# XiaRho/CMDA

Hardware: AMD Instinct MI355X
Metric: training images/sec (512x512 image+event, MiT-B5) (higher is better)
Workload: dtype bf16

## Files before the change

### cmda_amd/csrc/ce_loss.hip

```cpp
#include <cstdlib>
#include "bilinear.h"

namespace {
constexpr int kMaxClasses = 32;

template <int NC_MAX>
static __device__ __forceinline__ void upsample_scores(const float* __restrict__ lg, int b, int h, int w, int nc,
                                                       const BilinTap& ty, const BilinTap& tx, float (&s)[NC_MAX]) {
  const float* p00 = lg + ((long)(b * h + ty.i0) * w + tx.i0) * nc;
  const float* p01 = lg + ((long)(b * h + ty.i0) * w + tx.i1) * nc;
  const float* p10 = lg + ((long)(b * h + ty.i1) * w + tx.i0) * nc;
  const float* p11 = lg + ((long)(b * h + ty.i1) * w + tx.i1) * nc;
#pragma unroll
  for (int c = 0; c < NC_MAX; ++c)
    if (c < nc) s[c] = bilin_mix(p00[c], p01[c], p10[c], p11[c], tx.l0, tx.l1, ty.l0, ty.l1);
}

constexpr int kTW = 64, kTH = 8, kPatchFloats = 6144;

struct ScoreTile {
  int X0, Y0, b, tx0, ty0, ncols;
  bool staged;
};

static __device__ __forceinline__ ScoreTile stage_patch(const float* __restrict__ lg, float* __restrict__ patch, int h, int w, int H,
                                                        int W, int nc, float sh, float sw) {
  ScoreTile t;
  const int tiles_x = (W + kTW - 1) / kTW, tiles_y = (H + kTH - 1) / kTH;
  const int bt = blockIdx.x;
  t.b = bt / (tiles_x * tiles_y);
  const int r = bt - t.b * tiles_x * tiles_y;
  t.Y0 = (r / tiles_x) * kTH;
  t.X0 = (r % tiles_x) * kTW;
  const int X1 = min(t.X0 + kTW, W) - 1, Y1 = min(t.Y0 + kTH, H) - 1;
  t.tx0 = bilin_tap(t.X0, w, W, sw).i0;
  t.ty0 = bilin_tap(t.Y0, h, H, sh).i0;
  const int tx1 = bilin_tap(X1, w, W, sw).i1, ty1 = bilin_tap(Y1, h, H, sh).i1;
  t.ncols = tx1 - t.tx0 + 1;
  const int nrows = ty1 - t.ty0 + 1, rowf = t.ncols * nc;
  t.staged = rowf * nrows <= kPatchFloats;
  if (t.staged) {
    for (int rr = 0; rr < nrows; ++rr) {
      const float* src = lg + ((long)(t.b * h + t.ty0 + rr) * w + t.tx0) * nc;
      for (int k = threadIdx.x; k < rowf; k += blockDim.x) patch[rr * rowf + k] = src[k];
    }
  }
  __syncthreads();
  return t;
}

template <int NC_MAX>
static __device__ __forceinline__ void tile_scores(const ScoreTile& t, const float* __restrict__ lg, const float* __restrict__ patch,
                                                   int h, int w, int nc, const BilinTap& ty, const BilinTap& tx, float (&s)[NC_MAX]) {
  if (!t.staged) {
    upsample_scores<NC_MAX>(lg, t.b, h, w, nc, ty, tx, s);
    return;
  }
  const float* p00 = patch + ((ty.i0 - t.ty0) * t.ncols + (tx.i0 - t.tx0)) * nc;
  const float* p01 = patch + ((ty.i0 - t.ty0) * t.ncols + (tx.i1 - t.tx0)) * nc;
  const float* p10 = patch + ((ty.i1 - t.ty0) * t.ncols + (tx.i0 - t.tx0)) * nc;
  const float* p11 = patch + ((ty.i1 - t.ty0) * t.ncols + (tx.i1 - t.tx0)) * nc;
#pragma unroll
  for (int c = 0; c < NC_MAX; ++c)
    if (c < nc) s[c] = bilin_mix(p00[c], p01[c], p10[c], p11[c], tx.l0, tx.l1, ty.l0, ty.l1);
}

__global__ __launch_bounds__(256) void ce_fwd_kernel(const float* __restrict__ logits, const long long* __restrict__ label,
                                                      const float* __restrict__ weight, float* __restrict__ lse_out,
                                                      float* __restrict__ acc, int B, int h, int w, int H, int W, int nc,
                                                      int ignore_index) {
  __shared__ float red[2][4];
  __shared__ float patch[kPatchFloats];
  const float sh = (float)h / (float)H, sw = (float)w / (float)W;
  const ScoreTile t = stage_patch(logits, patch, h, w, H, W, nc, sh, sw);
  float lsum = 0.f, csum = 0.f;
  const int X = t.X0 + (threadIdx.x & (kTW - 1));
  for (int Y = t.Y0 + (threadIdx.x / kTW); Y < min(t.Y0 + kTH, H); Y += 256 / kTW) {
    if (X >= W) break;
    const long i = ((long)t.b * H + Y) * W + X;
    const BilinTap ty = bilin_tap(Y, h, H, sh), tx = bilin_tap(X, w, W, sw);
    float s[kMaxClasses];
    tile_scores<kMaxClasses>(t, logits, patch, h, w, nc, ty, tx, s);
    float mx = -INFINITY;
    int am = 0;
#pragma unroll
    for (int c = 0; c < kMaxClasses; ++c)
      if (c < nc && s[c] > mx) { mx = s[c]; am = c; }
    float se = 0.f;
#pragma unroll
    for (int c = 0; c < kMaxClasses; ++c)
      if (c < nc) se += __expf(s[c] - mx);
    const float lse = mx + __logf(se);
    if (lse_out) lse_out[i] = lse;
    const long long lab = label[i];
    if (lab != ignore_index && lab >= 0 && lab < nc) {
      float sl = 0.f;
#pragma unroll
      for (int c = 0; c < kMaxClasses; ++c)
        if (c == (int)lab) sl = s[c];
      const float wgt = weight ? weight[i] : 1.f;
      lsum += wgt * (lse - sl);
    }
    csum += ((long long)am == lab) ? 1.f : 0.f;
  }
  lsum = wave_sum(lsum);
  csum = wave_sum(csum);
  const int lane = threadIdx.x & 63, wid = threadIdx.x >> 6;
  if (lane == 0) { red[0][wid] = lsum; red[1][wid] = csum; }
  __syncthreads();
  if (threadIdx.x == 0) {
    atomicAdd(acc + 0, red[0][0] + red[0][1] + red[0][2] + red[0][3]);
    atomicAdd(acc + 1, red[1][0] + red[1][1] + red[1][2] + red[1][3]);
  }
}

__global__ void ce_bwd_kernel(const float* __restrict__ logits, const long long* __restrict__ label,
                              const float* __restrict__ weight, const float* __restrict__ lse,
                              const float* __restrict__ gscale_ptr, float gscale_mul, float* __restrict__ dlogits, int B,
                              int h, int w, int H, int W, int nc, int ignore_index) {
  const float sh = (float)h / (float)H, sw = (float)w / (float)W;
  const float ish = (float)H / (float)h, isw = (float)W / (float)w;
  const float gscale = (gscale_ptr ? *gscale_ptr : 1.f) * gscale_mul;
  const long total = (long)B * h * w;
  for (long i = (long)blockIdx.x * blockDim.x + threadIdx.x; i < total; i += (long)gridDim.x * blockDim.x) {
    const unsigned iu = (unsigned)i, tu = iu / (unsigned)w, bu = tu / (unsigned)h;
    const int x = (int)(iu - tu * (unsigned)w), y = (int)(tu - bu * (unsigned)h), b = (int)bu;
    int Y0 = (int)floorf(((float)y - 0.5f) * ish - 0.5f) - 1, Y1 = (int)ceilf(((float)y + 1.5f) * ish - 0.5f) + 1;
    int X0 = (int)floorf(((float)x - 0.5f) * isw - 0.5f) - 1, X1 = (int)ceilf(((float)x + 1.5f) * isw - 0.5f) + 1;
    if (y == 0) Y0 = 0;
    if (x == 0) X0 = 0;
    if (y == h - 1) Y1 = H - 1;
    if (x == w - 1) X1 = W - 1;
    Y0 = max(Y0, 0); X0 = max(X0, 0);
    Y1 = min(Y1, H - 1); X1 = min(X1, W - 1);
    float g[kMaxClasses];
#pragma unroll
    for (int c = 0; c < kMaxClasses; ++c) g[c] = 0.f;
    for (int Y = Y0; Y <= Y1; ++Y) {
      const BilinTap ty = bilin_tap(Y, h, H, sh);
      const float wy = (ty.i0 == y ? ty.l0 : 0.f) + (ty.i1 == y ? ty.l1 : 0.f);
      if (wy == 0.f) continue;
      for (int X = X0; X <= X1; ++X) {
        const BilinTap tx = bilin_tap(X, w, W, sw);
        const float wx = (tx.i0 == x ? tx.l0 : 0.f) + (tx.i1 == x ? tx.l1 : 0.f);
        if (wx == 0.f) continue;
        const long pi = ((long)b * H + Y) * W + X;
        const long long lab = label[pi];
        if (lab == ignore_index || lab < 0 || lab >= nc) continue;
        const float coef = wy * wx * (weight ? weight[pi] : 1.f);
        if (coef == 0.f) continue;
        float s[kMaxClasses];
        upsample_scores<kMaxClasses>(logits, b, h, w, nc, ty, tx, s);
        const float l = lse[pi];
#pragma unroll
        for (int c = 0; c < kMaxClasses; ++c)
          if (c < nc) g[c] += coef * (__expf(s[c] - l) - (c == (int)lab ? 1.f : 0.f));
      }
    }
    float* o = dlogits + i * nc;
#pragma unroll
    for (int c = 0; c < kMaxClasses; ++c)
      if (c < nc) o[c] = gscale * g[c];
  }
}

constexpr int kMaxTapsX = 16;

static __device__ __forceinline__ void lo_hi_range(int y, int h, int H, float ish, int& Y0, int& Y1) {
  Y0 = (int)floorf(((float)y - 0.5f) * ish - 0.5f) - 1;
  Y1 = (int)ceilf(((float)y + 1.5f) * ish - 0.5f) + 1;
  if (y == 0) Y0 = 0;
  if (y == h - 1) Y1 = H - 1;
  Y0 = max(Y0, 0);
  Y1 = min(Y1, H - 1);
}

static __device__ __forceinline__ void lo_hi_window(int y, int h, int H, float ish, int f, int& Y0, int& Y1) {
  if (f == 0) {
    lo_hi_range(y, h, H, ish, Y0, Y1);
    return;
  }
  Y0 = y == 0 ? 0 : f * y - (f >> 1);
  Y1 = y == h - 1 ? H - 1 : f * y + f + (f >> 1) - 1;
  Y0 = max(Y0, 0);
  Y1 = min(Y1, H - 1);
}

__global__ __launch_bounds__(256) void ce_bwd_gather_kernel(const float* __restrict__ logits, const long long* __restrict__ label,
                                                            const float* __restrict__ weight, const float* __restrict__ lse,
                                                            const float* __restrict__ gscale_ptr, float gscale_mul,
                                                            float* __restrict__ dlogits, int B, int h, int w, int H, int W,
                                                            int nc, int ignore_index) {
  const long total = (long)B * h * w * nc;
  const long i = (long)blockIdx.x * blockDim.x + threadIdx.x;
  if (i >= total) return;
  const float sh = (float)h / (float)H, sw = (float)w / (float)W;
  const float ish = (float)H / (float)h, isw = (float)W / (float)w;
  const unsigned iu = (unsigned)i, pu = iu / (unsigned)nc, tu = pu / (unsigned)w, bu = tu / (unsigned)h;
  const int c = (int)(iu - pu * (unsigned)nc), x = (int)(pu - tu * (unsigned)w), y = (int)(tu - bu * (unsigned)h), b = (int)bu;
  int Y0, Y1, X0, X1;
  lo_hi_range(y, h, H, ish, Y0, Y1);
  lo_hi_range(x, w, W, isw, X0, X1);
  float wxs[kMaxTapsX], lx0[kMaxTapsX], lx1[kMaxTapsX];
  unsigned sel0 = 0, sel1 = 0;
  const int nX = X1 - X0 + 1;
#pragma unroll
  for (int k = 0; k < kMaxTapsX; ++k) {
    wxs[k] = 0.f; lx0[k] = 0.f; lx1[k] = 0.f;
    if (k < nX) {
      const BilinTap tx = bilin_tap(X0 + k, w, W, sw);
      wxs[k] = (tx.i0 == x ? tx.l0 : 0.f) + (tx.i1 == x ? tx.l1 : 0.f);
      lx0[k] = tx.l0;
      lx1[k] = tx.l1;
      sel0 |= (tx.i0 == x ? 1u : 0u) << k;
      sel1 |= (tx.i1 == x ? 1u : 0u) << k;
    }
  }
  const int xm = max(x - 1, 0), xp = min(x + 1, w - 1);
  const float* Lb = logits + (long)b * h * w * nc + c;
  float g = 0.f;
  for (int Y = Y0; Y <= Y1; ++Y) {
    const BilinTap ty = bilin_tap(Y, h, H, sh);
    const float wy = (ty.i0 == y ? ty.l0 : 0.f) + (ty.i1 == y ? ty.l1 : 0.f);
    if (wy == 0.f) continue;
    const float* r0 = Lb + (long)ty.i0 * w * nc;
    const float* r1 = Lb + (long)ty.i1 * w * nc;
    const float a0 = r0[(long)xm * nc], a1 = r0[(long)x * nc], a2 = r0[(long)xp * nc];
    const float b0 = r1[(long)xm * nc], b1 = r1[(long)x * nc], b2 = r1[(long)xp * nc];
    const long rowp = ((long)b * H + Y) * W + X0;
#pragma unroll
    for (int k = 0; k < kMaxTapsX; ++k) {
      if (k >= nX || wxs[k] == 0.f) continue;
      const long long lab = label[rowp + k];
      if (lab == ignore_index || lab < 0 || lab >= nc) continue;
      const float coef = wy * wxs[k] * (weight ? weight[rowp + k] : 1.f);
      if (coef == 0.f) continue;
      const bool s0 = (sel0 >> k) & 1u, s1 = (sel1 >> k) & 1u;
      const float sc = bilin_mix(s0 ? a1 : a0, s1 ? a1 : a2, s0 ? b1 : b0, s1 ? b1 : b2, lx0[k], lx1[k], ty.l0, ty.l1);
      g += coef * (__expf(sc - lse[rowp + k]) - (c == (int)lab ? 1.f : 0.f));
    }
  }
  dlogits[i] = (gscale_ptr ? *gscale_ptr : 1.f) * gscale_mul * g;
}

constexpr int kTLW = 8, kTLH = 4, kStripRows = 8, kStripCols = 48, kStripFloats = kStripRows * kStripCols * 20;
constexpr int kLowPatchFloats = (kTLW + 6) * (kTLH + 6) * 20;

template <int NCT>
__global__ __launch_bounds__(320) void ce_bwd_tile_kernel(const float* __restrict__ logits, const long long* __restrict__ label,
                                                          const float* __restrict__ weight, const float* __restrict__ lse,
                                                          const float* __restrict__ gscale_ptr, float gscale_mul,
                                                          float* __restrict__ dlogits, int B, int h, int w, int H, int W,
                                                          int nc_rt, int ignore_index, int fy, int fx) {
  const int nc = NCT ? NCT : nc_rt;
  __shared__ float G[kStripFloats];
  __shared__ float patch[kLowPatchFloats];
  const float sh = (float)h / (float)H, sw = (float)w / (float)W;
  const float ish = (float)H / (float)h, isw = (float)W / (float)w;
  const int tiles_x = (w + kTLW - 1) / kTLW, tiles_y = (h + kTLH - 1) / kTLH;
  const int bt = blockIdx.x;
  const int b = bt / (tiles_x * tiles_y);
  const int r = bt - b * tiles_x * tiles_y;
  const int y0 = (r / tiles_x) * kTLH, x0 = (r % tiles_x) * kTLW;
  const int y1 = min(y0 + kTLH, h) - 1, x1 = min(x0 + kTLW, w) - 1;
  int YR0, YR1, XR0, XR1, tmp;
  lo_hi_window(y0, h, H, ish, fy, YR0, tmp);
  lo_hi_window(y1, h, H, ish, fy, tmp, YR1);
  lo_hi_window(x0, w, W, isw, fx, XR0, tmp);
  lo_hi_window(x1, w, W, isw, fx, tmp, XR1);
  const int ncols = XR1 - XR0 + 1;
  const int py0 = bilin_tap(YR0, h, H, sh).i0, py1 = bilin_tap(YR1, h, H, sh).i1;
  const int px0 = bilin_tap(XR0, w, W, sw).i0, px1 = bilin_tap(XR1, w, W, sw).i1;
  const int pcols = px1 - px0 + 1, prows = py1 - py0 + 1, prowf = pcols * nc;
  for (int rr = 0; rr < prows; ++rr) {
    const float* src = logits + ((long)(b * h + py0 + rr) * w + px0) * nc;
    for (int k = threadIdx.x; k < prowf; k += blockDim.x) patch[rr * prowf + k] = src[k];
  }
  const int per = kTLW * nc, ngrp = max(1, (int)blockDim.x / per), grp = threadIdx.x / per, tig = threadIdx.x - grp * per;
  const int gx = tig / nc, gc = tig - gx * nc;
  const bool gather = grp < ngrp && x0 + gx <= x1;
  const int x = x0 + gx;
  float wxs[kMaxTapsX];
  int X0 = 0, nX = 0;
  if (gather) {
    int X1;
    lo_hi_window(x, w, W, isw, fx, X0, X1);
    nX = X1 - X0 + 1;
  }
#pragma unroll
  for (int k = 0; k < kMaxTapsX; ++k) {
    wxs[k] = 0.f;
    if (k < nX) {
      const BilinTap tx = bilin_tap(X0 + k, w, W, sw);
      wxs[k] = (tx.i0 == x ? tx.l0 : 0.f) + (tx.i1 == x ? tx.l1 : 0.f);
    }
  }
  float acc[kTLH];
#pragma unroll
  for (int j = 0; j < kTLH; ++j) acc[j] = 0.f;
  __syncthreads();

  for (int YS = YR0; YS <= YR1; YS += kStripRows) {
    const int nrows = min(kStripRows, YR1 - YS + 1);
    for (int pi = threadIdx.x; pi < nrows * ncols; pi += blockDim.x) {
      const int ry = pi / ncols, rx = pi - ry * ncols;
      const int Y = YS + ry, X = XR0 + rx;
      float* gp = G + (ry * kStripCols + rx) * nc;
      const long gi = ((long)b * H + Y) * W + X;
      const long long lab = label[gi];
      const bool live = lab != ignore_index && lab >= 0 && lab < nc;
      const float coef = live ? (weight ? weight[gi] : 1.f) : 0.f;
      if (coef == 0.f) {
#pragma unroll
        for (int c = 0; c < (NCT ? NCT : kMaxClasses); ++c)
          if (c < nc) gp[c] = 0.f;
        continue;
      }
      const BilinTap ty = bilin_tap(Y, h, H, sh), tx = bilin_tap(X, w, W, sw);
      const float* p00 = patch + ((ty.i0 - py0) * pcols + (tx.i0 - px0)) * nc;
      const float* p01 = patch + ((ty.i0 - py0) * pcols + (tx.i1 - px0)) * nc;
      const float* p10 = patch + ((ty.i1 - py0) * pcols + (tx.i0 - px0)) * nc;
      const float* p11 = patch + ((ty.i1 - py0) * pcols + (tx.i1 - px0)) * nc;
      const float l = lse[gi];
#pragma unroll
      for (int c = 0; c < (NCT ? NCT : kMaxClasses); ++c) {
        if (c < nc) {
          const float sc = bilin_mix(p00[c], p01[c], p10[c], p11[c], tx.l0, tx.l1, ty.l0, ty.l1);
          gp[c] = coef * (__expf(sc - l) - (c == (int)lab ? 1.f : 0.f));
        }
      }
    }
    __syncthreads();
    if (gather) {
      for (int ry = grp; ry < nrows; ry += ngrp) {
        const BilinTap ty = bilin_tap(YS + ry, h, H, sh);
        const float* gr = G + (ry * kStripCols + (X0 - XR0)) * nc + gc;
        float t = 0.f;
#pragma unroll
        for (int k = 0; k < kMaxTapsX; ++k)
          if (k < nX) t += wxs[k] * gr[k * nc];
#pragma unroll
        for (int j = 0; j < kTLH; ++j) {
          const int y = y0 + j;
          const float wy = (ty.i0 == y ? ty.l0 : 0.f) + (ty.i1 == y ? ty.l1 : 0.f);
          acc[j] += wy * t;
        }
      }
    }
    __syncthreads();
  }
  if (ngrp > 1) {
    if (gather && grp > 0) {
#pragma unroll
      for (int j = 0; j < kTLH; ++j) G[((grp - 1) * per + tig) * kTLH + j] = acc[j];
    }
    __syncthreads();
    if (gather && grp == 0) {
      for (int o = 1; o < ngrp; ++o)
#pragma unroll
        for (int j = 0; j < kTLH; ++j) acc[j] += G[((o - 1) * per + tig) * kTLH + j];
    }
  }
  if (!gather || grp != 0) return;
  const float gs = (gscale_ptr ? *gscale_ptr : 1.f) * gscale_mul;
#pragma unroll
  for (int j = 0; j < kTLH; ++j) {
    const int y = y0 + j;
    if (y <= y1) dlogits[(((long)b * h + y) * w + x) * nc + gc] = gs * acc[j];
  }
}

__global__ __launch_bounds__(256) void pseudo_label_kernel(const float* __restrict__ logits, long long* __restrict__ label_out,
                                                            float* __restrict__ prob_out, int* __restrict__ count, int B, int h, int w,
                                                            int H, int W, int nc, float thr) {
  __shared__ int red[4];
  __shared__ float patch[kPatchFloats];
  const float sh = (float)h / (float)H, sw = (float)w / (float)W;
  const ScoreTile t = stage_patch(logits, patch, h, w, H, W, nc, sh, sw);
  int cnt = 0;
  const int X = t.X0 + (threadIdx.x & (kTW - 1));
  for (int Y = t.Y0 + (threadIdx.x / kTW); Y < min(t.Y0 + kTH, H); Y += 256 / kTW) {
    if (X >= W) break;
    const long i = ((long)t.b * H + Y) * W + X;
    const BilinTap ty = bilin_tap(Y, h, H, sh), tx = bilin_tap(X, w, W, sw);
    float s[kMaxClasses];
    tile_scores<kMaxClasses>(t, logits, patch, h, w, nc, ty, tx, s);
    float mx = -INFINITY;
    int am = 0;
#pragma unroll
    for (int c = 0; c < kMaxClasses; ++c)
      if (c < nc && s[c] > mx) { mx = s[c]; am = c; }
    float se = 0.f;
#pragma unroll
    for (int c = 0; c < kMaxClasses; ++c)
      if (c < nc) se += __expf(s[c] - mx);
    const float prob = 1.f / se;
    label_out[i] = am;
    if (prob_out) prob_out[i] = prob;
    cnt += prob >= thr ? 1 : 0;
  }
  float cf = wave_sum((float)cnt);
  const int lane = threadIdx.x & 63, wid = threadIdx.x >> 6;
  if (lane == 0) red[wid] = (int)cf;
  __syncthreads();
  if (threadIdx.x == 0) atomicAdd(count, red[0] + red[1] + red[2] + red[3]);
}

__global__ void upsample_logits_nchw_kernel(const float* __restrict__ logits, float* __restrict__ out, int B, int h,
                                            int w, int H, int W, int nc) {
  const float sh = (float)h / (float)H, sw = (float)w / (float)W;
  const long total = (long)B * H * W;
  for (long i = (long)blockIdx.x * blockDim.x + threadIdx.x; i < total; i += (long)gridDim.x * blockDim.x) {
    const unsigned iu = (unsigned)i, tu = iu / (unsigned)W, bu = tu / (unsigned)H;
    const int X = (int)(iu - tu * (unsigned)W), Y = (int)(tu - bu * (unsigned)H), b = (int)bu;
    const BilinTap ty = bilin_tap(Y, h, H, sh), tx = bilin_tap(X, w, W, sw);
    float s[kMaxClasses];
    upsample_scores<kMaxClasses>(logits, b, h, w, nc, ty, tx, s);
#pragma unroll
    for (int c = 0; c < kMaxClasses; ++c)
      if (c < nc) out[(((long)b * nc + c) * H + Y) * W + X] = s[c];
  }
}

__global__ void pseudo_weight_kernel(const int* __restrict__ count, float* __restrict__ weight, int B, int H, int W,
                                     int top, int bottom) {
  const long total = (long)B * H * W;
  const float v = (float)((double)(*count) / (double)total);
  for (long i = (long)blockIdx.x * blockDim.x + threadIdx.x; i < total; i += (long)gridDim.x * blockDim.x) {
    const int Y = (int)((i / W) % H);
    weight[i] = (Y < top || Y >= H - bottom) ? 0.f : v;
  }
}

static inline int grid_for(long n) { return (int)std::max<long>(1, std::min<long>((n + 255) / 256, 4096)); }
}

extern "C" int cmda_ce_upsample_fwd(const float* logits, const int64_t* label, const float* weight, float* lse_out,
                                    float* acc, int B, int h, int w, int H, int W, int nc, int ignore_index,
                                    void* stream) {
  if ((long)B * H * W <= 0) return CMDA_OK;
  if (nc <= 0 || nc > kMaxClasses) return CMDA_ERR_SHAPE;
  const long tiles = (long)B * ((W + kTW - 1) / kTW) * ((H + kTH - 1) / kTH);
  if (tiles > 0x7fffffffL) return CMDA_ERR_SHAPE;
  CMDA_LAUNCH(ce_fwd_kernel, dim3((unsigned)tiles), dim3(256), 0, stream, logits, (const long long*)label, weight, lse_out, acc, B, h,
              w, H, W, nc, ignore_index);
  CMDA_CHECK_LAUNCH();
}

extern "C" int cmda_ce_upsample_bwd(const float* logits, const int64_t* label, const float* weight, const float* lse,
                                    const float* gscale_ptr, float gscale_mul, float* dlogits, int B, int h, int w,
                                    int H, int W, int nc, int ignore_index, void* stream) {
  if ((long)B * h * w <= 0) return CMDA_OK;
  if (nc <= 0 || nc > kMaxClasses) return CMDA_ERR_SHAPE;
  if ((long)B * h * w * nc >= (1L << 32)) return CMDA_ERR_SHAPE;
  const long taps = (long)ceil(2.0 * W / w) + 4;
  {
    const long rcols = (long)ceil((kTLW + 1.0) * W / w) + 6;
    if (taps <= kMaxTapsX && 2L * h <= H && 2L * w <= W && rcols <= kStripCols && nc <= 20 && getenv("CMDA_CE_GATHER") == nullptr) {
      const long tiles = (long)B * ((w + kTLW - 1) / kTLW) * ((h + kTLH - 1) / kTLH);
      if (tiles > 0x7fffffffL) return CMDA_ERR_SHAPE;
      auto pow2_factor = [](int out, int in) { const int f = out / in; return (out % in) == 0 && f >= 2 && f <= 16 && (f & (f - 1)) == 0 ? f : 0; };
      const int fy = pow2_factor(H, h), fx = pow2_factor(W, w);
      if (nc == 19) CMDA_LAUNCH(ce_bwd_tile_kernel<19>, dim3((unsigned)tiles), dim3(320), 0, stream, logits, (const long long*)label, weight, lse, gscale_ptr,
                                gscale_mul, dlogits, B, h, w, H, W, nc, ignore_index, fy, fx);
      else CMDA_LAUNCH(ce_bwd_tile_kernel<0>, dim3((unsigned)tiles), dim3(320), 0, stream, logits, (const long long*)label, weight, lse, gscale_ptr,
                       gscale_mul, dlogits, B, h, w, H, W, nc, ignore_index, fy, fx);
      CMDA_CHECK_LAUNCH();
    }
  }
  if (taps <= kMaxTapsX && h <= H && w <= W) {
    const long blocks = ((long)B * h * w * nc + 255) / 256;
    if (blocks > 0x7fffffffL) return CMDA_ERR_SHAPE;
    CMDA_LAUNCH(ce_bwd_gather_kernel, dim3((unsigned)blocks), dim3(256), 0, stream, logits, (const long long*)label, weight, lse,
                gscale_ptr, gscale_mul, dlogits, B, h, w, H, W, nc, ignore_index);
    CMDA_CHECK_LAUNCH();
  }
  CMDA_LAUNCH(ce_bwd_kernel, dim3(grid_for((long)B * h * w)), dim3(256), 0, stream, logits, (const long long*)label,
              weight, lse, gscale_ptr, gscale_mul, dlogits, B, h, w, H, W, nc, ignore_index);
  CMDA_CHECK_LAUNCH();
}

extern "C" int cmda_pseudo_label(const float* logits, int64_t* label_out, float* prob_out, int* count, int B, int h,
                                 int w, int H, int W, int nc, float thr, void* stream) {
  if ((long)B * H * W <= 0) return CMDA_OK;
  if (nc <= 0 || nc > kMaxClasses) return CMDA_ERR_SHAPE;
  const long tiles = (long)B * ((W + kTW - 1) / kTW) * ((H + kTH - 1) / kTH);
  if (tiles > 0x7fffffffL) return CMDA_ERR_SHAPE;
  CMDA_LAUNCH(pseudo_label_kernel, dim3((unsigned)tiles), dim3(256), 0, stream, logits, (long long*)label_out, prob_out, count, B, h,
              w, H, W, nc, thr);
  CMDA_CHECK_LAUNCH();
}

extern "C" int cmda_pseudo_weight(const int* count, float* weight, int B, int H, int W, int top, int bottom,
                                  void* stream) {
  if ((long)B * H * W <= 0) return CMDA_OK;
  CMDA_LAUNCH(pseudo_weight_kernel, dim3(grid_for((long)B * H * W)), dim3(256), 0, stream, count, weight, B, H, W, top,
              bottom);
  CMDA_CHECK_LAUNCH();
}

extern "C" int cmda_upsample_logits_nchw(const float* logits, float* out, int B, int h, int w, int H, int W, int nc,
                                         void* stream) {
  if ((long)B * H * W <= 0) return CMDA_OK;
  if (nc <= 0 || nc > kMaxClasses) return CMDA_ERR_SHAPE;
  if ((long)B * H * W >= (1L << 32)) return CMDA_ERR_SHAPE;
  CMDA_LAUNCH(upsample_logits_nchw_kernel, dim3(grid_for((long)B * H * W)), dim3(256), 0, stream, logits, out, B, h, w,
              H, W, nc);
  CMDA_CHECK_LAUNCH();
}
```

Measured before the change: 39.90.

## Restructure CE forward, backward and pseudo-label kernels with vectorized tiles

The CE forward and pseudo-label kernels become persistent 512-thread blocks that loop over tiles. Each thread handles four pixels, with vectorized label, weight and LSE loads and stores, and a 19-class specialization pads rows to 20 so staged patches can be read as float4. The backward tile kernel moves to dynamic shared memory, stages through a batched multi-load helper, and prefetches the next strip's labels, weights and LSE into registers. These changes target global-memory latency and launch overhead, at the cost of more registers, more code paths and a larger shared-memory footprint.

```diff
diff --git a/cmda_amd/csrc/ce_loss.hip b/cmda_amd/csrc/ce_loss.hip
--- a/cmda_amd/csrc/ce_loss.hip
+++ b/cmda_amd/csrc/ce_loss.hip
@@ -16,101 +16,215 @@
     if (c < nc) s[c] = bilin_mix(p00[c], p01[c], p10[c], p11[c], tx.l0, tx.l1, ty.l0, ty.l1);
 }
 
-constexpr int kTW = 64, kTH = 8, kPatchFloats = 6144;
+constexpr int kCeThreads = 512, kTW = 64, kTH = 4 * kCeThreads / kTW, kPatchFloats = 6144, kStageDepth = 8;
+constexpr int kCeMaxBlocks = 256;
+
+struct alignas(16) I64x2 { long long x, y; };
 
 struct ScoreTile {
   int X0, Y0, b, tx0, ty0, ncols;
   bool staged;
 };
 
-static __device__ __forceinline__ ScoreTile stage_patch(const float* __restrict__ lg, float* __restrict__ patch, int h, int w, int H,
-                                                        int W, int nc, float sh, float sw) {
+template <int NCT, int THREADS>
+static __device__ __forceinline__ void stage_lowres(const float* __restrict__ src, float* __restrict__ patch, int nrows, int ncols, int w,
+                                                    int nc) {
+  constexpr bool kPad = NCT == 19;
+  const int rowl = ncols * (kPad ? 20 : nc), total = rowl * nrows;
+  const float inv_rowl = 1.f / (float)rowl;
+  for (int k0 = threadIdx.x; k0 < total; k0 += kStageDepth * THREADS) {
+    float v[kStageDepth];
+#pragma unroll
+    for (int j = 0; j < kStageDepth; ++j) {
+      const int k = k0 + j * THREADS;
+      v[j] = 0.f;
+      if (k < total) {
+        int rr = (int)((float)k * inv_rowl);
+        if (rr * rowl > k) --rr;
+        if ((rr + 1) * rowl <= k) ++rr;
+        const int e = k - rr * rowl;
+        if (kPad) {
+          const int cc = e / 20, c = e - cc * 20;
+          if (c < 19) v[j] = src[(long)rr * w * nc + cc * 19 + c];
+        } else {
+          v[j] = src[(long)rr * w * nc + e];
+        }
+      }
+    }
+#pragma unroll
+    for (int j = 0; j < kStageDepth; ++j) {
+      const int k = k0 + j * THREADS;
+      if (k < total) patch[k] = v[j];
+    }
+  }
+}
+
+static __device__ __forceinline__ ScoreTile tile_origin(int tile, int H, int W) {
   ScoreTile t;
   const int tiles_x = (W + kTW - 1) / kTW, tiles_y = (H + kTH - 1) / kTH;
-  const int bt = blockIdx.x;
-  t.b = bt / (tiles_x * tiles_y);
-  const int r = bt - t.b * tiles_x * tiles_y;
+  t.b = tile / (tiles_x * tiles_y);
+  const int r = tile - t.b * tiles_x * tiles_y;
   t.Y0 = (r / tiles_x) * kTH;
   t.X0 = (r % tiles_x) * kTW;
+  t.tx0 = t.ty0 = t.ncols = 0;
+  t.staged = false;
+  return t;
+}
+
+template <int NCT>
+static __device__ __forceinline__ void stage_patch(ScoreTile& t, const float* __restrict__ lg, float* __restrict__ patch, int h, int w,
+                                                   int H, int W, int nc, float sh, float sw) {
+  constexpr bool kPad = NCT == 19;
+  const int ps = kPad ? 20 : nc;
   const int X1 = min(t.X0 + kTW, W) - 1, Y1 = min(t.Y0 + kTH, H) - 1;
   t.tx0 = bilin_tap(t.X0, w, W, sw).i0;
   t.ty0 = bilin_tap(t.Y0, h, H, sh).i0;
   const int tx1 = bilin_tap(X1, w, W, sw).i1, ty1 = bilin_tap(Y1, h, H, sh).i1;
   t.ncols = tx1 - t.tx0 + 1;
-  const int nrows = ty1 - t.ty0 + 1, rowf = t.ncols * nc;
-  t.staged = rowf * nrows <= kPatchFloats;
-  if (t.staged) {
-    for (int rr = 0; rr < nrows; ++rr) {
-      const float* src = lg + ((long)(t.b * h + t.ty0 + rr) * w + t.tx0) * nc;
-      for (int k = threadIdx.x; k < rowf; k += blockDim.x) patch[rr * rowf + k] = src[k];
-    }
-  }
-  __syncthreads();
-  return t;
-}
-
-template <int NC_MAX>
+  const int nrows = ty1 - t.ty0 + 1;
+  t.staged = t.ncols * ps * nrows <= kPatchFloats;
+  if (t.staged) stage_lowres<NCT, kCeThreads>(lg + ((long)(t.b * h + t.ty0) * w + t.tx0) * nc, patch, nrows, t.ncols, w, nc);
+}
+
+template <int NCT>
 static __device__ __forceinline__ void tile_scores(const ScoreTile& t, const float* __restrict__ lg, const float* __restrict__ patch,
-                                                   int h, int w, int nc, const BilinTap& ty, const BilinTap& tx, float (&s)[NC_MAX]) {
+                                                   int h, int w, int nc, const BilinTap& ty, const BilinTap& tx,
+                                                   float (&s)[NCT ? 20 : kMaxClasses]) {
   if (!t.staged) {
-    upsample_scores<NC_MAX>(lg, t.b, h, w, nc, ty, tx, s);
+    upsample_scores<(NCT ? 20 : kMaxClasses)>(lg, t.b, h, w, nc, ty, tx, s);
     return;
   }
-  const float* p00 = patch + ((ty.i0 - t.ty0) * t.ncols + (tx.i0 - t.tx0)) * nc;
-  const float* p01 = patch + ((ty.i0 - t.ty0) * t.ncols + (tx.i1 - t.tx0)) * nc;
-  const float* p10 = patch + ((ty.i1 - t.ty0) * t.ncols + (tx.i0 - t.tx0)) * nc;
-  const float* p11 = patch + ((ty.i1 - t.ty0) * t.ncols + (tx.i1 - t.tx0)) * nc;
-#pragma unroll
-  for (int c = 0; c < NC_MAX; ++c)
-    if (c < nc) s[c] = bilin_mix(p00[c], p01[c], p10[c], p11[c], tx.l0, tx.l1, ty.l0, ty.l1);
-}
-
-__global__ __launch_bounds__(256) void ce_fwd_kernel(const float* __restrict__ logits, const long long* __restrict__ label,
-                                                      const float* __restrict__ weight, float* __restrict__ lse_out,
-                                                      float* __restrict__ acc, int B, int h, int w, int H, int W, int nc,
-                                                      int ignore_index) {
-  __shared__ float red[2][4];
-  __shared__ float patch[kPatchFloats];
+  const int ps = NCT == 19 ? 20 : nc;
+  const float* p00 = patch + ((ty.i0 - t.ty0) * t.ncols + (tx.i0 - t.tx0)) * ps;
+  const float* p01 = patch + ((ty.i0 - t.ty0) * t.ncols + (tx.i1 - t.tx0)) * ps;
+  const float* p10 = patch + ((ty.i1 - t.ty0) * t.ncols + (tx.i0 - t.tx0)) * ps;
+  const float* p11 = patch + ((ty.i1 - t.ty0) * t.ncols + (tx.i1 - t.tx0)) * ps;
+  if (NCT == 19) {
+#pragma unroll
+    for (int v = 0; v < 5; ++v) {
+      const float4 a = reinterpret_cast<const float4*>(p00)[v], b = reinterpret_cast<const float4*>(p01)[v];
+      const float4 c = reinterpret_cast<const float4*>(p10)[v], d = reinterpret_cast<const float4*>(p11)[v];
+      s[4 * v + 0] = bilin_mix(a.x, b.x, c.x, d.x, tx.l0, tx.l1, ty.l0, ty.l1);
+      s[4 * v + 1] = bilin_mix(a.y, b.y, c.y, d.y, tx.l0, tx.l1, ty.l0, ty.l1);
+      s[4 * v + 2] = bilin_mix(a.z, b.z, c.z, d.z, tx.l0, tx.l1, ty.l0, ty.l1);
+      s[4 * v + 3] = bilin_mix(a.w, b.w, c.w, d.w, tx.l0, tx.l1, ty.l0, ty.l1);
+    }
+  } else {
+#pragma unroll
+    for (int c = 0; c < kMaxClasses; ++c)
+      if (c < nc) s[c] = bilin_mix(p00[c], p01[c], p10[c], p11[c], tx.l0, tx.l1, ty.l0, ty.l1);
+  }
+}
+
+template <int NCT>
+static __device__ __forceinline__ void score_stats(const float (&s)[NCT ? 20 : kMaxClasses], int nc, float& mx, int& am, float& se) {
+  constexpr int kN = NCT ? NCT : kMaxClasses;
+  mx = -INFINITY;
+  am = 0;
+#pragma unroll
+  for (int c = 0; c < kN; ++c)
+    if (c < nc && s[c] > mx) { mx = s[c]; am = c; }
+  se = 0.f;
+#pragma unroll
+  for (int c = 0; c < kN; ++c)
+    if (c < nc) se += __expf(s[c] - mx);
+}
+
+struct Quad {
+  int X, Y;
+  long i;
+  bool row, all;
+};
+static __device__ __forceinline__ Quad tile_quad(const ScoreTile& t, int H, int W) {
+  Quad q;
+  q.X = t.X0 + 4 * (threadIdx.x & (kTW / 4 - 1));
+  q.Y = t.Y0 + threadIdx.x / (kTW / 4);
+  q.row = q.Y < H && q.X < W;
+  q.all = q.row && q.X + 3 < W;
+  q.i = ((long)t.b * H + q.Y) * W + q.X;
+  return q;
+}
+
+template <int NCT>
+__global__ __launch_bounds__(kCeThreads) void ce_fwd_kernel(const float* __restrict__ logits, const long long* __restrict__ label,
+                                                             const float* __restrict__ weight, float* __restrict__ lse_out,
+                                                             float* __restrict__ acc, int B, int h, int w, int H, int W, int nc_rt,
+                                                             int ignore_index, int tiles, int vec) {
+  const int nc = NCT ? NCT : nc_rt;
+  __shared__ float red[2][kCeThreads / 64];
+  __shared__ __attribute__((aligned(16))) float patch[kPatchFloats];
   const float sh = (float)h / (float)H, sw = (float)w / (float)W;
-  const ScoreTile t = stage_patch(logits, patch, h, w, H, W, nc, sh, sw);
   float lsum = 0.f, csum = 0.f;
-  const int X = t.X0 + (threadIdx.x & (kTW - 1));
-  for (int Y = t.Y0 + (threadIdx.x / kTW); Y < min(t.Y0 + kTH, H); Y += 256 / kTW) {
-    if (X >= W) break;
-    const long i = ((long)t.b * H + Y) * W + X;
-    const BilinTap ty = bilin_tap(Y, h, H, sh), tx = bilin_tap(X, w, W, sw);
-    float s[kMaxClasses];
-    tile_scores<kMaxClasses>(t, logits, patch, h, w, nc, ty, tx, s);
-    float mx = -INFINITY;
-    int am = 0;
-#pragma unroll
-    for (int c = 0; c < kMaxClasses; ++c)
-      if (c < nc && s[c] > mx) { mx = s[c]; am = c; }
-    float se = 0.f;
-#pragma unroll
-    for (int c = 0; c < kMaxClasses; ++c)
-      if (c < nc) se += __expf(s[c] - mx);
-    const float lse = mx + __logf(se);
-    if (lse_out) lse_out[i] = lse;
-    const long long lab = label[i];
-    if (lab != ignore_index && lab >= 0 && lab < nc) {
-      float sl = 0.f;
-#pragma unroll
-      for (int c = 0; c < kMaxClasses; ++c)
-        if (c == (int)lab) sl = s[c];
-      const float wgt = weight ? weight[i] : 1.f;
-      lsum += wgt * (lse - sl);
-    }
-    csum += ((long long)am == lab) ? 1.f : 0.f;
+  for (int tile = blockIdx.x; tile < tiles; tile += gridDim.x) {
+    ScoreTile t = tile_origin(tile, H, W);
+    const Quad q = tile_quad(t, H, W);
+    long long lab[4];
+    float wgt[4] = {1.f, 1.f, 1.f, 1.f};
+    if (vec && q.all) {
+      const I64x2 l0 = *reinterpret_cast<const I64x2*>(label + q.i), l1 = *reinterpret_cast<const I64x2*>(label + q.i + 2);
+      lab[0] = l0.x; lab[1] = l0.y; lab[2] = l1.x; lab[3] = l1.y;
+      if (weight) {
+        const float4 wv = *reinterpret_cast<const float4*>(weight + q.i);
+        wgt[0] = wv.x; wgt[1] = wv.y; wgt[2] = wv.z; wgt[3] = wv.w;
+      }
+    } else {
+#pragma unroll
+      for (int j = 0; j < 4; ++j) {
+        const bool in = q.row && q.X + j < W;
+        lab[j] = in ? label[q.i + j] : (long long)ignore_index;
+        if (in && weight) wgt[j] = weight[q.i + j];
+      }
+    }
+    stage_patch<NCT>(t, logits, patch, h, w, H, W, nc, sh, sw);
+    __syncthreads();
+    if (q.row) {
+      const BilinTap ty = bilin_tap(q.Y, h, H, sh);
+      float lv[4];
+#pragma unroll
+      for (int j = 0; j < 4; ++j) {
+        lv[j] = 0.f;
+        if (q.X + j < W) {
+          const BilinTap tx = bilin_tap(q.X + j, w, W, sw);
+          float s[NCT ? 20 : kMaxClasses];
+          tile_scores<NCT>(t, logits, patch, h, w, nc, ty, tx, s);
+          float mx, se;
+          int am;
+          score_stats<NCT>(s, nc, mx, am, se);
+          const float lse = mx + __logf(se);
+          lv[j] = lse;
+          const long long lb = lab[j];
+          if (lb != ignore_index && lb >= 0 && lb < nc) {
+            float sl = 0.f;
+#pragma unroll
+            for (int c = 0; c < (NCT ? NCT : kMaxClasses); ++c)
+              if (c == (int)lb) sl = s[c];
+            lsum += wgt[j] * (lse - sl);
+          }
+          csum += ((long long)am == lb) ? 1.f : 0.f;
+        }
+      }
+      if (lse_out) {
+        if (vec && q.all) {
+          *reinterpret_cast<float4*>(lse_out + q.i) = make_float4(lv[0], lv[1], lv[2], lv[3]);
+        } else {
+#pragma unroll
+          for (int j = 0; j < 4; ++j)
+            if (q.X + j < W) lse_out[q.i + j] = lv[j];
+        }
+      }
+    }
+    __syncthreads();
   }
   lsum = wave_sum(lsum);
   csum = wave_sum(csum);
   const int lane = threadIdx.x & 63, wid = threadIdx.x >> 6;
   if (lane == 0) { red[0][wid] = lsum; red[1][wid] = csum; }
   __syncthreads();
-  if (threadIdx.x == 0) {
-    atomicAdd(acc + 0, red[0][0] + red[0][1] + red[0][2] + red[0][3]);
-    atomicAdd(acc + 1, red[1][0] + red[1][1] + red[1][2] + red[1][3]);
+  if (threadIdx.x < 2) {
+    float v = 0.f;
+#pragma unroll
+    for (int k = 0; k < kCeThreads / 64; ++k) v += red[threadIdx.x][k];
+    atomicAdd(acc + threadIdx.x, v);
   }
 }
 
@@ -243,18 +357,45 @@
   dlogits[i] = (gscale_ptr ? *gscale_ptr : 1.f) * gscale_mul * g;
 }
 
-constexpr int kTLW = 8, kTLH = 4, kStripRows = 8, kStripCols = 48, kStripFloats = kStripRows * kStripCols * 20;
-constexpr int kLowPatchFloats = (kTLW + 6) * (kTLH + 6) * 20;
+constexpr int kTLW = 8, kTLH = 4, kStripRows = 8, kStripCols = 48, kBwdThreads = 320;
+constexpr int kStripPix = (kStripRows * kStripCols + kBwdThreads - 1) / kBwdThreads;
+
+struct StripIn {
+  long long lab[kStripPix];
+  float wgt[kStripPix], lse[kStripPix];
+};
+
+static __device__ __forceinline__ void strip_fetch(StripIn& in, const long long* __restrict__ label, const float* __restrict__ weight,
+                                                   const float* __restrict__ lse, int b, int H, int W, int YS, int YR1, int XR0,
+                                                   int ncols, int ignore_index) {
+  const int nrows = min(kStripRows, YR1 - YS + 1);
+#pragma unroll
+  for (int j = 0; j < kStripPix; ++j) {
+    const int pi = threadIdx.x + j * kBwdThreads;
+    in.lab[j] = ignore_index;
+    in.wgt[j] = 1.f;
+    in.lse[j] = 0.f;
+    if (pi < nrows * ncols) {
+      const int ry = pi / ncols, rx = pi - ry * ncols;
+      const long gi = ((long)b * H + YS + ry) * W + XR0 + rx;
+      in.lab[j] = label[gi];
+      if (weight) in.wgt[j] = weight[gi];
+      in.lse[j] = lse[gi];
+    }
+  }
+}
 
 template <int NCT>
-__global__ __launch_bounds__(320) void ce_bwd_tile_kernel(const float* __restrict__ logits, const long long* __restrict__ label,
-                                                          const float* __restrict__ weight, const float* __restrict__ lse,
-                                                          const float* __restrict__ gscale_ptr, float gscale_mul,
-                                                          float* __restrict__ dlogits, int B, int h, int w, int H, int W,
-                                                          int nc_rt, int ignore_index, int fy, int fx) {
+__global__ __launch_bounds__(kBwdThreads) void ce_bwd_tile_kernel(const float* __restrict__ logits, const long long* __restrict__ label,
+                                                                   const float* __restrict__ weight, const float* __restrict__ lse,
+                                                                   const float* __restrict__ gscale_ptr, float gscale_mul,
+                                                                   float* __restrict__ dlogits, int B, int h, int w, int H, int W,
+                                                                   int nc_rt, int ignore_index, int fy, int fx, int gcols, int vecst) {
   const int nc = NCT ? NCT : nc_rt;
-  __shared__ float G[kStripFloats];
-  __shared__ float patch[kLowPatchFloats];
+  const int ps = NCT == 19 ? 20 : nc;
+  CMDA_DYN_SMEM(smem);
+  float* G = reinterpret_cast<float*>(smem);
+  float* patch = G + kStripRows * gcols * 20;
   const float sh = (float)h / (float)H, sw = (float)w / (float)W;
   const float ish = (float)H / (float)h, isw = (float)W / (float)w;
   const int tiles_x = (w + kTLW - 1) / kTLW, tiles_y = (h + kTLH - 1) / kTLH;
@@ -269,14 +410,13 @@
   lo_hi_window(x0, w, W, isw, fx, XR0, tmp);
   lo_hi_window(x1, w, W, isw, fx, tmp, XR1);
   const int ncols = XR1 - XR0 + 1;
+  StripIn nxt;
+  strip_fetch(nxt, label, weight, lse, b, H, W, YR0, YR1, XR0, ncols, ignore_index);
   const int py0 = bilin_tap(YR0, h, H, sh).i0, py1 = bilin_tap(YR1, h, H, sh).i1;
   const int px0 = bilin_tap(XR0, w, W, sw).i0, px1 = bilin_tap(XR1, w, W, sw).i1;
-  const int pcols = px1 - px0 + 1, prows = py1 - py0 + 1, prowf = pcols * nc;
-  for (int rr = 0; rr < prows; ++rr) {
-    const float* src = logits + ((long)(b * h + py0 + rr) * w + px0) * nc;
-    for (int k = threadIdx.x; k < prowf; k += blockDim.x) patch[rr * prowf + k] = src[k];
-  }
-  const int per = kTLW * nc, ngrp = max(1, (int)blockDim.x / per), grp = threadIdx.x / per, tig = threadIdx.x - grp * per;
+  const int pcols = px1 - px0 + 1, prows = py1 - py0 + 1;
+  stage_lowres<NCT, kBwdThreads>(logits + ((long)(b * h + py0) * w + px0) * nc, patch, prows, pcols, w, nc);
+  const int per = kTLW * nc, ngrp = max(1, kBwdThreads / per), grp = threadIdx.x / per, tig = threadIdx.x - grp * per;
   const int gx = tig / nc, gc = tig - gx * nc;
   const bool gather = grp < ngrp && x0 + gx <= x1;
   const int x = x0 + gx;
@@ -302,31 +442,58 @@
 
   for (int YS = YR0; YS <= YR1; YS += kStripRows) {
     const int nrows = min(kStripRows, YR1 - YS + 1);
-    for (int pi = threadIdx.x; pi < nrows * ncols; pi += blockDim.x) {
+    const StripIn cur = nxt;
+    if (YS + kStripRows <= YR1) strip_fetch(nxt, label, weight, lse, b, H, W, YS + kStripRows, YR1, XR0, ncols, ignore_index);
+#pragma unroll
+    for (int j = 0; j < kStripPix; ++j) {
+      const int pi = threadIdx.x + j * kBwdThreads;
+      if (pi >= nrows * ncols) continue;
       const int ry = pi / ncols, rx = pi - ry * ncols;
       const int Y = YS + ry, X = XR0 + rx;
-      float* gp = G + (ry * kStripCols + rx) * nc;
-      const long gi = ((long)b * H + Y) * W + X;
-      const long long lab = label[gi];
+      float* gp = G + (ry * gcols + rx) * ps;
+      const long long lab = cur.lab[j];
       const bool live = lab != ignore_index && lab >= 0 && lab < nc;
-      const float coef = live ? (weight ? weight[gi] : 1.f) : 0.f;
+      const float coef = live ? cur.wgt[j] : 0.f;
       if (coef == 0.f) {
-#pragma unroll
-        for (int c = 0; c < (NCT ? NCT : kMaxClasses); ++c)
-          if (c < nc) gp[c] = 0.f;
+        if (NCT == 19) {
+#pragma unroll
+          for (int v = 0; v < 5; ++v) reinterpret_cast<float4*>(gp)[v] = make_float4(0.f, 0.f, 0.f, 0.f);
+        } else {
+#pragma unroll
+          for (int c = 0; c < kMaxClasses; ++c)
+            if (c < nc) gp[c] = 0.f;
+        }
         continue;
       }
       const BilinTap ty = bilin_tap(Y, h, H, sh), tx = bilin_tap(X, w, W, sw);
-      const float* p00 = patch + ((ty.i0 - py0) * pcols + (tx.i0 - px0)) * nc;
-      const float* p01 = patch + ((ty.i0 - py0) * pcols + (tx.i1 - px0)) * nc;
-      const float* p10 = patch + ((ty.i1 - py0) * pcols + (tx.i0 - px0)) * nc;
-      const float* p11 = patch + ((ty.i1 - py0) * pcols + (tx.i1 - px0)) * nc;
-      const float l = lse[gi];
-#pragma unroll
-      for (int c = 0; c < (NCT ? NCT : kMaxClasses); ++c) {
-        if (c < nc) {
-          const float sc = bilin_mix(p00[c], p01[c], p10[c], p11[c], tx.l0, tx.l1, ty.l0, ty.l1);
-          gp[c] = coef * (__expf(sc - l) - (c == (int)lab ? 1.f : 0.f));
+      const float* p00 = patch + ((ty.i0 - py0) * pcols + (tx.i0 - px0)) * ps;
+      const float* p01 = patch + ((ty.i0 - py0) * pcols + (tx.i1 - px0)) * ps;
+      const float* p10 = patch + ((ty.i1 - py0) * pcols + (tx.i0 - px0)) * ps;
+      const float* p11 = patch + ((ty.i1 - py0) * pcols + (tx.i1 - px0)) * ps;
+      const float l = cur.lse[j];
+      if (NCT == 19) {
+#pragma unroll
+        for (int v = 0; v < 5; ++v) {
+          const float4 a4 = reinterpret_cast<const float4*>(p00)[v], b4 = reinterpret_cast<const float4*>(p01)[v];
+          const float4 c4 = reinterpret_cast<const float4*>(p10)[v], d4 = reinterpret_cast<const float4*>(p11)[v];
+          const float av[4] = {a4.x, a4.y, a4.z, a4.w}, bv[4] = {b4.x, b4.y, b4.z, b4.w};
+          const float cv[4] = {c4.x, c4.y, c4.z, c4.w}, dv[4] = {d4.x, d4.y, d4.z, d4.w};
+          float o[4];
+#pragma unroll
+          for (int e = 0; e < 4; ++e) {
+            const int c = 4 * v + e;
+            const float sc = bilin_mix(av[e], bv[e], cv[e], dv[e], tx.l0, tx.l1, ty.l0, ty.l1);
+            o[e] = c < 19 ? coef * (__expf(sc - l) - (c == (int)lab ? 1.f : 0.f)) : 0.f;
+          }
+          reinterpret_cast<float4*>(gp)[v] = make_float4(o[0], o[1], o[2], o[3]);
+        }
+      } else {
+#pragma unroll
+        for (int c = 0; c < kMaxClasses; ++c) {
+          if (c < nc) {
+            const float sc = bilin_mix(p00[c], p01[c], p10[c], p11[c], tx.l0, tx.l1, ty.l0, ty.l1);
+            gp[c] = coef * (__expf(sc - l) - (c == (int)lab ? 1.f : 0.f));
+          }
         }
       }
     }
@@ -334,11 +501,11 @@
     if (gather) {
       for (int ry = grp; ry < nrows; ry += ngrp) {
         const BilinTap ty = bilin_tap(YS + ry, h, H, sh);
-        const float* gr = G + (ry * kStripCols + (X0 - XR0)) * nc + gc;
+        const float* gr = G + (ry * gcols + (X0 - XR0)) * ps + gc;
         float t = 0.f;
 #pragma unroll
         for (int k = 0; k < kMaxTapsX; ++k)
-          if (k < nX) t += wxs[k] * gr[k * nc];
+          if (k < nX) t += wxs[k] * gr[k * ps];
 #pragma unroll
         for (int j = 0; j < kTLH; ++j) {
           const int y = y0 + j;
@@ -349,61 +516,98 @@
     }
     __syncthreads();
   }
-  if (ngrp > 1) {
-    if (gather && grp > 0) {
-#pragma unroll
-      for (int j = 0; j < kTLH; ++j) G[((grp - 1) * per + tig) * kTLH + j] = acc[j];
-    }
+  float* F = G;
+  if (gather) {
+#pragma unroll
+    for (int j = 0; j < kTLH; ++j) F[(grp * kTLH + j) * per + tig] = acc[j];
+  }
+  __syncthreads();
+  const float gs = (gscale_ptr ? *gscale_ptr : 1.f) * gscale_mul;
+  const int rowl = (x1 - x0 + 1) * nc, ny = y1 - y0 + 1;
+  if (vecst && (rowl & 3) == 0) {
+    const int rv = rowl >> 2;
+    for (int k = threadIdx.x; k < ny * rv; k += kBwdThreads) {
+      const int j = k / rv, v = k - j * rv;
+      float4 a = *reinterpret_cast<const float4*>(F + j * per + 4 * v);
+      for (int o = 1; o < ngrp; ++o) {
+        const float4 c = *reinterpret_cast<const float4*>(F + (o * kTLH + j) * per + 4 * v);
+        a.x += c.x; a.y += c.y; a.z += c.z; a.w += c.w;
+      }
+      *reinterpret_cast<float4*>(dlogits + (((long)b * h + y0 + j) * w + x0) * nc + 4 * v) = make_float4(gs * a.x, gs * a.y, gs * a.z, gs * a.w);
+    }
+  } else {
+    for (int k = threadIdx.x; k < ny * rowl; k += kBwdThreads) {
+      const int j = k / rowl, e = k - j * rowl;
+      float a = F[j * per + e];
+      for (int o = 1; o < ngrp; ++o) a += F[(o * kTLH + j) * per + e];
+      dlogits[(((long)b * h + y0 + j) * w + x0) * nc + e] = gs * a;
+    }
+  }
+}
+
+template <int NCT>
+__global__ __launch_bounds__(kCeThreads) void pseudo_label_kernel(const float* __restrict__ logits, long long* __restrict__ label_out,
+                                                                   float* __restrict__ prob_out, int* __restrict__ count, int B, int h,
+                                                                   int w, int H, int W, int nc_rt, float thr, int tiles, int vec) {
+  const int nc = NCT ? NCT : nc_rt;
+  __shared__ int red[kCeThreads / 64];
+  __shared__ __attribute__((aligned(16))) float patch[kPatchFloats];
+  const float sh = (float)h / (float)H, sw = (float)w / (float)W;
+  int cnt = 0;
+  for (int tile = blockIdx.x; tile < tiles; tile += gridDim.x) {
+    ScoreTile t = tile_origin(tile, H, W);
+    stage_patch<NCT>(t, logits, patch, h, w, H, W, nc, sh, sw);
     __syncthreads();
-    if (gather && grp == 0) {
-      for (int o = 1; o < ngrp; ++o)
-#pragma unroll
-        for (int j = 0; j < kTLH; ++j) acc[j] += G[((o - 1) * per + tig) * kTLH + j];
-    }
-  }
-  if (!gather || grp != 0) return;
-  const float gs = (gscale_ptr ? *gscale_ptr : 1.f) * gscale_mul;
-#pragma unroll
-  for (int j = 0; j < kTLH; ++j) {
-    const int y = y0 + j;
-    if (y <= y1) dlogits[(((long)b * h + y) * w + x) * nc + gc] = gs * acc[j];
-  }
-}
-
-__global__ __launch_bounds__(256) void pseudo_label_kernel(const float* __restrict__ logits, long long* __restrict__ label_out,
-                                                            float* __restrict__ prob_out, int* __restrict__ count, int B, int h, int w,
-                                                            int H, int W, int nc, float thr) {
-  __shared__ int red[4];
-  __shared__ float patch[kPatchFloats];
-  const float sh = (float)h / (float)H, sw = (float)w / (float)W;
-  const ScoreTile t = stage_patch(logits, patch, h, w, H, W, nc, sh, sw);
-  int cnt = 0;
-  const int X = t.X0 + (threadIdx.x & (kTW - 1));
-  for (int Y = t.Y0 + (threadIdx.x / kTW); Y < min(t.Y0 + kTH, H); Y += 256 / kTW) {
-    if (X >= W) break;
-    const long i = ((long)t.b * H + Y) * W + X;
-    const BilinTap ty = bilin_tap(Y, h, H, sh), tx = bilin_tap(X, w, W, sw);
-    float s[kMaxClasses];
-    tile_scores<kMaxClasses>(t, logits, patch, h, w, nc, ty, tx, s);
-    float mx = -INFINITY;
-    int am = 0;
-#pragma unroll
-    for (int c = 0; c < kMaxClasses; ++c)
-      if (c < nc && s[c] > mx) { mx = s[c]; am = c; }
-    float se = 0.f;
-#pragma unroll
-    for (int c = 0; c < kMaxClasses; ++c)
-      if (c < nc) se += __expf(s[c] - mx);
-    const float prob = 1.f / se;
-    label_out[i] = am;
-    if (prob_out) prob_out[i] = prob;
-    cnt += prob >= thr ? 1 : 0;
-  }
-  float cf = wave_sum((float)cnt);
+    const Quad q = tile_quad(t, H, W);
+    if (q.row) {
+      const BilinTap ty = bilin_tap(q.Y, h, H, sh);
+      long long lv[4];
+      float pv[4];
+#pragma unroll
+      for (int j = 0; j < 4; ++j) {
+        lv[j] = 0;
+        pv[j] = 0.f;
+        if (q.X + j < W) {
+          const BilinTap tx = bilin_tap(q.X + j, w, W, sw);
+          float s[NCT ? 20 : kMaxClasses];
+          tile_scores<NCT>(t, logits, patch, h, w, nc, ty, tx, s);
+          float mx, se;
+          int am;
+          score_stats<NCT>(s, nc, mx, am, se);
+          const float prob = 1.f / se;
+          lv[j] = am;
+          pv[j] = prob;
+          cnt += prob >= thr ? 1 : 0;
+        }
+      }
+      if (vec && q.all) {
+        I64x2 a, b;
+        a.x = lv[0]; a.y = lv[1]; b.x = lv[2]; b.y = lv[3];
+        *reinterpret_cast<I64x2*>(label_out + q.i) = a;
+        *reinterpret_cast<I64x2*>(label_out + q.i + 2) = b;
+        if (prob_out) *reinterpret_cast<float4*>(prob_out + q.i) = make_float4(pv[0], pv[1], pv[2], pv[3]);
+      } else {
+#pragma unroll
+        for (int j = 0; j < 4; ++j) {
+          if (q.X + j < W) {
+            label_out[q.i + j] = lv[j];
+            if (prob_out) prob_out[q.i + j] = pv[j];
+          }
+        }
+      }
+    }
+    __syncthreads();
+  }
+  const float cf = wave_sum((float)cnt);
   const int lane = threadIdx.x & 63, wid = threadIdx.x >> 6;
   if (lane == 0) red[wid] = (int)cf;
   __syncthreads();
-  if (threadIdx.x == 0) atomicAdd(count, red[0] + red[1] + red[2] + red[3]);
+  if (threadIdx.x == 0) {
+    int v = 0;
+#pragma unroll
+    for (int k = 0; k < kCeThreads / 64; ++k) v += red[k];
+    atomicAdd(count, v);
+  }
 }
 
 __global__ void upsample_logits_nchw_kernel(const float* __restrict__ logits, float* __restrict__ out, int B, int h,
@@ -432,6 +636,7 @@
   }
 }
 
+static inline bool aligned16(const void* p) { return ((uintptr_t)p & 15) == 0; }
 static inline int grid_for(long n) { return (int)std::max<long>(1, std::min<long>((n + 255) / 256, 4096)); }
 }
 
@@ -442,8 +647,12 @@
   if (nc <= 0 || nc > kMaxClasses) return CMDA_ERR_SHAPE;
   const long tiles = (long)B * ((W + kTW - 1) / kTW) * ((H + kTH - 1) / kTH);
   if (tiles > 0x7fffffffL) return CMDA_ERR_SHAPE;
-  CMDA_LAUNCH(ce_fwd_kernel, dim3((unsigned)tiles), dim3(256), 0, stream, logits, (const long long*)label, weight, lse_out, acc, B, h,
-              w, H, W, nc, ignore_index);
+  const int vec = W % 4 == 0 && aligned16(label) && aligned16(weight) && aligned16(lse_out);
+  const dim3 grid((unsigned)std::min<long>(tiles, kCeMaxBlocks));
+  if (nc == 19) CMDA_LAUNCH(ce_fwd_kernel<19>, grid, dim3(kCeThreads), 0, stream, logits, (const long long*)label, weight, lse_out, acc, B, h,
+                            w, H, W, nc, ignore_index, (int)tiles, vec);
+  else CMDA_LAUNCH(ce_fwd_kernel<0>, grid, dim3(kCeThreads), 0, stream, logits, (const long long*)label, weight, lse_out, acc, B, h,
+                   w, H, W, nc, ignore_index, (int)tiles, vec);
   CMDA_CHECK_LAUNCH();
 }
 
@@ -461,10 +670,14 @@
       if (tiles > 0x7fffffffL) return CMDA_ERR_SHAPE;
       auto pow2_factor = [](int out, int in) { const int f = out / in; return (out % in) == 0 && f >= 2 && f <= 16 && (f & (f - 1)) == 0 ? f : 0; };
       const int fy = pow2_factor(H, h), fx = pow2_factor(W, w);
-      if (nc == 19) CMDA_LAUNCH(ce_bwd_tile_kernel<19>, dim3((unsigned)tiles), dim3(320), 0, stream, logits, (const long long*)label, weight, lse, gscale_ptr,
-                                gscale_mul, dlogits, B, h, w, H, W, nc, ignore_index, fy, fx);
-      else CMDA_LAUNCH(ce_bwd_tile_kernel<0>, dim3((unsigned)tiles), dim3(320), 0, stream, logits, (const long long*)label, weight, lse, gscale_ptr,
-                       gscale_mul, dlogits, B, h, w, H, W, nc, ignore_index, fy, fx);
+      const int gcols = fx ? (kTLW + 1) * fx : (int)rcols;
+      const int pcells = (kTLW + (fx ? 3 : 6)) * (kTLH + (fy ? 3 : 6));
+      const size_t smem = (size_t)(kStripRows * gcols + pcells) * 20 * sizeof(float);
+      const int vecst = aligned16(dlogits) && ((long)w * nc) % 4 == 0;
+      if (nc == 19) CMDA_LAUNCH(ce_bwd_tile_kernel<19>, dim3((unsigned)tiles), dim3(kBwdThreads), smem, stream, logits, (const long long*)label, weight, lse,
+                                gscale_ptr, gscale_mul, dlogits, B, h, w, H, W, nc, ignore_index, fy, fx, gcols, vecst);
+      else CMDA_LAUNCH(ce_bwd_tile_kernel<0>, dim3((unsigned)tiles), dim3(kBwdThreads), smem, stream, logits, (const long long*)label, weight, lse,
+                       gscale_ptr, gscale_mul, dlogits, B, h, w, H, W, nc, ignore_index, fy, fx, gcols, vecst);
       CMDA_CHECK_LAUNCH();
     }
   }
@@ -486,8 +699,12 @@
   if (nc <= 0 || nc > kMaxClasses) return CMDA_ERR_SHAPE;
   const long tiles = (long)B * ((W + kTW - 1) / kTW) * ((H + kTH - 1) / kTH);
   if (tiles > 0x7fffffffL) return CMDA_ERR_SHAPE;
-  CMDA_LAUNCH(pseudo_label_kernel, dim3((unsigned)tiles), dim3(256), 0, stream, logits, (long long*)label_out, prob_out, count, B, h,
-              w, H, W, nc, thr);
+  const int vec = W % 4 == 0 && aligned16(label_out) && aligned16(prob_out);
+  const dim3 grid((unsigned)std::min<long>(tiles, kCeMaxBlocks));
+  if (nc == 19) CMDA_LAUNCH(pseudo_label_kernel<19>, grid, dim3(kCeThreads), 0, stream, logits, (long long*)label_out, prob_out, count, B, h,
+                            w, H, W, nc, thr, (int)tiles, vec);
+  else CMDA_LAUNCH(pseudo_label_kernel<0>, grid, dim3(kCeThreads), 0, stream, logits, (long long*)label_out, prob_out, count, B, h,
+                   w, H, W, nc, thr, (int)tiles, vec);
   CMDA_CHECK_LAUNCH();
 }
 
```

Result: no change. 40.14, median of 6 (+0.6%).
